# Enter-tainer/oavif

Hardware: AMD Instinct MI355X
Metric: ssimulacra2_megapixels_per_sec (higher is better)
Workload: dtype f32; 1 GPU; ssimulacra2 score of one 3840x2160 RGB8 (ref, dist) pair per step per GPU (BASELINE configs[1]); steps rotate over 16 distinct pairs per GPU = 796 MB of frames resident in HBM (> the 256 MiB Infinity Cache); width=3840, height=2160, distinct_pairs_per_gpu=16, parallelism=single gpu, streams_per_gpu=2

## Files before the change

### include/ssimu2_hip_internal.h

```cpp
#ifndef SSIMU2_HIP_INTERNAL_H_
#define SSIMU2_HIP_INTERNAL_H_

#include "ssimu2_hip.h"

#ifdef __cplusplus
extern "C" {
#endif
#if defined(__GNUC__)
#pragma GCC visibility push(default)
#endif

enum { SSIMU2_DEBUG_LIN_REF = 0, SSIMU2_DEBUG_LIN_DIST = 1, SSIMU2_DEBUG_XYB_REF = 2, SSIMU2_DEBUG_REF_BLUR = 3,
       SSIMU2_DEBUG_RG_H = 4, SSIMU2_DEBUG_RG_V = 5 };
int ssimu2_debug_download(ssimu2_ctx* ctx, int what, int scale, uint32_t w, uint32_t h, float* out,
                          uint32_t* out_w, uint32_t* out_h);

int ssimu2_time_device(ssimu2_ctx* ctx, const void* d_ref, const void* d_dist, uint32_t w,
                       uint32_t h, int iters, float* out_ms_total, double* out_score);

enum { SSIMU2_STAGE_PYRAMID = 0, SSIMU2_STAGE_MARCH = 1, SSIMU2_STAGE_FINALIZE = 2 };
int ssimu2_time_stage(ssimu2_ctx* ctx, const void* d_ref, const void* d_dist, uint32_t w, uint32_t h,
                      int stage, int iters, float* out_ms_avg);

int ssimu2_time_march_rotating(ssimu2_ctx* ctx, const void* const* d_refs, const void* const* d_dists,
                               int npairs, uint32_t w, uint32_t h, int iters, float* out_ms_avg);

int ssimu2_measure_read_stream(ssimu2_ctx* ctx, size_t bytes, int iters, double* out_gbps);

int ssimu2_instr_set_segment_rows(ssimu2_ctx* ctx, int rows_scale0, int rows_other_scales);
int ssimu2_instr_cache_reference_blur(ssimu2_ctx* ctx, int enabled);
enum {
    SSIMU2_MARCH_NONE = 0,
    SSIMU2_MARCH_PAIR_U8 = 1,
    SSIMU2_MARCH_REFBLUR_U8 = 2,
    SSIMU2_MARCH_PAIR_LIN = 3,
    SSIMU2_MARCH_REFBLUR_LIN = 4,
    SSIMU2_MARCH_PAIR_BATCH = 5,
    SSIMU2_MARCH_REFBLUR_BATCH = 6
};
int ssimu2_instr_last_march(ssimu2_ctx* ctx, int* out_kind);
int ssimu2_instr_set_batch_segment_rows(ssimu2_ctx* ctx, int rows_scale0);
int ssimu2_instr_batch_segment_rows(ssimu2_ctx* ctx, uint32_t w, uint32_t h, int scale, int* out_rows);
int ssimu2_time_blur_stage_rotating(ssimu2_ctx* ctx, const void* const* d_frames, int nframes, uint32_t w,
                                    uint32_t h, int iters, float* out_ms_avg, double* out_bytes_per_launch);
int ssimu2_time_kernels(ssimu2_ctx* ctx, const void* d_ref, const void* const* d_refs, const void* const* d_dists, int n,
                        uint32_t w, uint32_t h, int iters, float* out_ms_avg, int* out_launches, float* out_ms_wall_timed,
                        float* out_ms_wall_plain);
int ssimu2_instr_placed_streams(ssimu2_ctx* ctx, int* out_n);
int ssimu2_instr_rg_stop_after_scale(ssimu2_ctx* ctx, int scale);

#if defined(__GNUC__)
#pragma GCC visibility pop
#endif
#ifdef __cplusplus
}
#endif
#endif
```

### oavif_amd/csrc/ssimu2_instrument.hip

```cpp
#define SSIMU2_INSTRUMENTED_BUILD 1
#include "ssimu2_hip.hip"

#include <vector>

#include "../../include/ssimu2_hip_internal.h"

namespace ssimu2 {

__global__ __launch_bounds__(256) void k_read_stream(const uint4* __restrict__ src, size_t n16,
                                                     uint32_t* __restrict__ sink) {
    const size_t chunk = (n16 + gridDim.x - 1) / gridDim.x;
    const size_t lo = (size_t)blockIdx.x * chunk;
    const size_t hi = lo + chunk < n16 ? lo + chunk : n16;
    size_t i = lo + threadIdx.x;
    uint4 acc = make_uint4(0, 0, 0, 0);
    for (; i + 768 < hi; i += 1024) {
        const uint4 a = src[i], b = src[i + 256], c = src[i + 512], d = src[i + 768];
        acc.x ^= a.x ^ b.x ^ c.x ^ d.x;
        acc.y ^= a.y ^ b.y ^ c.y ^ d.y;
        acc.z ^= a.z ^ b.z ^ c.z ^ d.z;
        acc.w ^= a.w ^ b.w ^ c.w ^ d.w;
    }
    for (; i < hi; i += 256) {
        const uint4 a = src[i];
        acc.x ^= a.x; acc.y ^= a.y; acc.z ^= a.z; acc.w ^= a.w;
    }
    const uint32_t v = acc.x ^ acc.y ^ acc.z ^ acc.w;
    if (v == 0x9E3779B9u) *sink = v;
}

}

extern "C" {

int ssimu2_instr_set_segment_rows(ssimu2_ctx* c, int rows_scale0, int rows_other_scales) {
    REMOTE_REFUSE(c, "ssimu2_instr_set_segment_rows");
    if (!c) return SSIMU2_ERR_INVALID_ARG;
    if ((rows_scale0 != 0 && (rows_scale0 < 8 || rows_scale0 > 160)) ||
        (rows_other_scales != 0 && (rows_other_scales < 8 || rows_other_scales > 160)))
        return c->fail(SSIMU2_ERR_INVALID_ARG, "segment rows must be 0 (default rule) or 8..160");
    HIP_TRY(c, hipSetDevice(c->device));
    HIP_TRY(c, hipStreamSynchronize(c->stream));
    c->seg_rows_override = rows_scale0;
    c->seg_rows_tail_override = rows_other_scales;
    release_frame_groups(c);
    return SSIMU2_OK;
}

int ssimu2_instr_set_batch_segment_rows(ssimu2_ctx* c, int rows_scale0) {
    REMOTE_REFUSE(c, "ssimu2_instr_set_batch_segment_rows");
    if (!c) return SSIMU2_ERR_INVALID_ARG;
    if (rows_scale0 != 0 && rows_scale0 != -1 && (rows_scale0 < 8 || rows_scale0 > 160))
        return c->fail(SSIMU2_ERR_INVALID_ARG, "batch segment rows must be 0 (the rule), -1 (the single-score rule) or 8..160");
    HIP_TRY(c, hipSetDevice(c->device));
    HIP_TRY(c, hipStreamSynchronize(c->stream));
    c->batch_seg_override = rows_scale0;
    return SSIMU2_OK;
}

int ssimu2_instr_batch_segment_rows(ssimu2_ctx* c, uint32_t w, uint32_t h, int scale, int* out_rows) {
    REMOTE_REFUSE(c, "ssimu2_instr_batch_segment_rows");
    if (!c || !out_rows || scale < 0 || scale >= kNumScales || w == 0 || h == 0) return SSIMU2_ERR_INVALID_ARG;
    *out_rows = batch_seg_rows(c, make_pyramid(w, h), scale);
    return SSIMU2_OK;
}

int ssimu2_instr_placed_streams(ssimu2_ctx* c, int* out_n) {
    REMOTE_REFUSE(c, "ssimu2_instr_placed_streams");
    if (!c || !out_n) return SSIMU2_ERR_INVALID_ARG;
    *out_n = pool_size(c->device);
    return SSIMU2_OK;
}

int ssimu2_instr_rg_stop_after_scale(ssimu2_ctx* c, int scale) {
    REMOTE_REFUSE(c, "ssimu2_instr_rg_stop_after_scale");
    if (!c) return SSIMU2_ERR_INVALID_ARG;
    c->rg_dbg_scale = scale < 0 || scale >= kNumScales ? -1 : scale;
    return SSIMU2_OK;
}

int ssimu2_instr_cache_reference_blur(ssimu2_ctx* c, int enabled) {
    REMOTE_REFUSE(c, "ssimu2_instr_cache_reference_blur");
    if (!c) return SSIMU2_ERR_INVALID_ARG;
    c->cache_ref_blur = enabled != 0;
    c->ref.drop();
    return SSIMU2_OK;
}

int ssimu2_instr_last_march(ssimu2_ctx* c, int* out_kind) {
    REMOTE_REFUSE(c, "ssimu2_instr_last_march");
    if (!c || !out_kind) return SSIMU2_ERR_INVALID_ARG;
    *out_kind = c->last_march;
    return SSIMU2_OK;
}

int ssimu2_debug_download(ssimu2_ctx* c, int what, int scale, uint32_t w, uint32_t h, float* out,
                          uint32_t* out_w, uint32_t* out_h) {
    REMOTE_REFUSE(c, "ssimu2_debug_download");
    if (!c || !out) return SSIMU2_ERR_INVALID_ARG;
    if (w == 0 || h == 0) return c->fail(SSIMU2_ERR_INVALID_ARG, "zero image dimension");
    const Pyramid p = make_pyramid(w, h);
    const float* src = nullptr;
    if ((what == SSIMU2_DEBUG_LIN_REF || what == SSIMU2_DEBUG_LIN_DIST) && scale == 0) {
        const bool r = what == SSIMU2_DEBUG_LIN_REF;
        const void* planes = r ? c->hbd.lin0_ref.p : c->hbd.lin0_dist.p;
        if (!planes || p.nscales < 1 || (r ? c->lin0_ref_w : c->lin0_dist_w) != w ||
            (r ? c->lin0_ref_h : c->lin0_dist_h) != h)
            return c->fail(SSIMU2_ERR_INVALID_ARG, "no 16-bit scale-0 planes of that frame from the last score");
        src = (const float*)planes;
    } else if (what == SSIMU2_DEBUG_LIN_REF || what == SSIMU2_DEBUG_LIN_DIST) {
        if (scale < 1 || scale >= p.nscales || !c->frame.lin_ref.p) return c->fail(SSIMU2_ERR_INVALID_ARG, "no such level");
        src = (what == SSIMU2_DEBUG_LIN_REF ? c->frame.lin_ref : c->frame.lin_dist).as<float>() + p.lin_off[scale];
    } else if (what == SSIMU2_DEBUG_XYB_REF) {
        if (scale < 0 || scale >= p.nscales || !c->cache.xyb.p || !c->ref.have || c->ref.w != w || c->ref.h != h)
            return c->fail(SSIMU2_ERR_INVALID_ARG, "no cached reference XYB for that level");
        src = c->cache.xyb.as<float>() + xyb_off(p, scale);
    } else if (what == SSIMU2_DEBUG_RG_H || what == SSIMU2_DEBUG_RG_V) {
        if (scale < 0 || scale >= p.nscales || scale != c->rg_dbg_scale || !c->rg.dbg.p || !c->rg.planes.p)
            return c->fail(SSIMU2_ERR_INVALID_ARG, "no recursive-blur planes kept for that scale");
        const size_t pitch = (size_t)rg_pitch(p.w[scale]), wd = (size_t)p.w[scale], ht = (size_t)p.h[scale];
        const size_t nd = pitch * ht, n1 = wd * ht;
        if (24 * nd * sizeof(float) > c->rg.dbg.cap) return c->fail(SSIMU2_ERR_INVALID_ARG, "recursive-blur planes are of another frame size");
        HIP_TRY(c, hipSetDevice(c->device));
        HIP_TRY(c, hipStreamSynchronize(c->stream));
        auto plane = [&](float* dst, const float* src) {
            return hipMemcpy2D(dst, wd * sizeof(float), src, pitch * sizeof(float), wd * sizeof(float), ht, hipMemcpyDeviceToHost);
        };
        if (what == SSIMU2_DEBUG_RG_H) {
            for (int k = 0; k < 15; ++k) HIP_TRY(c, plane(out + (size_t)k * n1, c->rg.dbg.as<float>() + (size_t)k * nd));
        } else {
            const float* cache = c->rg.planes.as<float>() + 6 * rg_plane_off(p, p.nscales) + 6 * rg_plane_off(p, scale);
            const float* pass = c->rg.dbg.as<float>() + 15 * nd;
            for (int ch = 0; ch < 3; ++ch) {
                for (int k = 0; k < 2; ++k)
                    HIP_TRY(c, plane(out + (size_t)rg_plane15(true, ch, k) * n1, cache + (size_t)(ch * 2 + k) * nd));
                for (int k = 0; k < 3; ++k)
                    HIP_TRY(c, plane(out + (size_t)rg_plane15(false, ch, k) * n1, pass + (size_t)(ch * 3 + k) * nd));
            }
        }
        if (out_w) *out_w = (uint32_t)p.w[scale];
        if (out_h) *out_h = (uint32_t)p.h[scale];
        return SSIMU2_OK;
    } else if (what == SSIMU2_DEBUG_REF_BLUR) {
        if (scale < 0 || scale >= p.nscales || !c->cache.blur.p || !c->ref.have || c->ref.w != w || c->ref.h != h)
            return c->fail(SSIMU2_ERR_INVALID_ARG, "no cached reference blur for that level");
        src = c->cache.blur.as<float>() + xyb_off(p, scale);
    } else {
        return c->fail(SSIMU2_ERR_INVALID_ARG, "bad `what`");
    }
    HIP_TRY(c, hipSetDevice(c->device));
    HIP_TRY(c, hipStreamSynchronize(c->stream));
    const size_t n = (size_t)3 * p.w[scale] * p.h[scale];
    HIP_TRY(c, hipMemcpy(out, src, n * sizeof(float), hipMemcpyDeviceToHost));
    if (out_w) *out_w = (uint32_t)p.w[scale];
    if (out_h) *out_h = (uint32_t)p.h[scale];
    return SSIMU2_OK;
}

int ssimu2_time_device(ssimu2_ctx* c, const void* d_ref, const void* d_dist, uint32_t w,
                       uint32_t h, int iters, float* out_ms_total, double* out_score) {
    REMOTE_REFUSE(c, "ssimu2_time_device");
    int rc = check_args(c, d_ref, d_dist, w, h);
    if (rc) return rc;
    if (iters <= 0 || !out_ms_total) return c->fail(SSIMU2_ERR_INVALID_ARG, "bad iters/out");
    HIP_TRY(c, hipSetDevice(c->device));
    if ((rc = ensure_capacity(c, w, h))) return rc;
    c->ref.drop();
    HIP_TRY(c, hipEventRecord(c->ev0, c->stream));
    for (int i = 0; i < iters; ++i)
        if ((rc = enqueue_score(c, (const uint8_t*)d_ref, (const uint8_t*)d_dist, w, h, false)))
            return rc;
    HIP_TRY(c, hipEventRecord(c->ev1, c->stream));
    double score = 0.0;
    if ((rc = ssimu2_wait(c, &score))) return rc;
    HIP_TRY(c, hipEventSynchronize(c->ev1));
    HIP_TRY(c, hipEventElapsedTime(out_ms_total, c->ev0, c->ev1));
    if (out_score) *out_score = score;
    return SSIMU2_OK;
}

}

namespace {

template <class F>
struct AtExit {
    F f;
    ~AtExit() { f(); }
};
template <class F>
AtExit(F) -> AtExit<F>;
auto scratch_guard(ssimu2_ctx* c, DevBuf& b) {
    return AtExit{[c, &b] { (void)hipStreamSynchronize(c->stream), b.release(); }};
}

template <class T>
std::vector<T> host_array(int n) {
    try {
        return std::vector<T>((size_t)n);
    } catch (const std::bad_alloc&) {
        return {};
    }
}

template <class F>
hipError_t timed_loop(ssimu2_ctx* c, int warm, int iters, float* ms, F&& fn) {
    for (int j = 0; j < warm; ++j) fn(j);
    hipError_t e = hipEventRecord(c->ev0, c->stream);
    for (int j = 0; j < iters && e == hipSuccess; ++j) fn(j);
    if (e == hipSuccess) e = hipEventRecord(c->ev1, c->stream);
    if (e == hipSuccess) e = hipGetLastError();
    if (e == hipSuccess) e = hipEventSynchronize(c->ev1);
    if (e == hipSuccess) e = hipEventElapsedTime(ms, c->ev0, c->ev1);
    return e;
}

}

extern "C" {

int ssimu2_time_stage(ssimu2_ctx* c, const void* d_ref, const void* d_dist, uint32_t w, uint32_t h,
                      int stage, int iters, float* out_ms_avg) {
    REMOTE_REFUSE(c, "ssimu2_time_stage");
    int rc = check_args(c, d_ref, d_dist, w, h);
    if (rc) return rc;
    if (iters <= 0 || !out_ms_avg) return c->fail(SSIMU2_ERR_INVALID_ARG, "bad iters/out");
    double score;
    if ((rc = ssimu2_score_rgb8_device(c, d_ref, d_dist, w, h, &score))) return rc;
    const Pyramid p = make_pyramid(w, h);
    MarchPlan mp;
    FinalizeArgs fa;
    const int blocks = build_plans(c, p, march_seg_rows, score_sources(c, d_ref, d_dist, false), &mp, &fa);
    if (stage < 0 || stage > 2) return c->fail(SSIMU2_ERR_INVALID_ARG, "bad stage");
    const uint8_t* frames[2] = {(const uint8_t*)d_ref, (const uint8_t*)d_dist};
    float* lin[2] = {c->frame.lin_ref.as<float>(), c->frame.lin_dist.as<float>()};
    float ms = 0.f;
    const hipError_t e = timed_loop(c, 0, iters, &ms, [&](int) {
        if (stage == SSIMU2_STAGE_PYRAMID) launch_pyramid(c, p, 2, frames, lin);
        else if (stage == SSIMU2_STAGE_FINALIZE) launch(k_finalize, dim3(1), dim3(1024), 0, c->stream, fa, c->d_result);
        else if (blocks > 0) launch(k_march, dim3(blocks), dim3(MARCH_THREADS), 0, c->stream, mp);
    });
    if (e != hipSuccess) return c->fail(SSIMU2_ERR_HIP, "stage timing", e);
    *out_ms_avg = ms / (float)iters;
    return SSIMU2_OK;
}

int ssimu2_time_march_rotating(ssimu2_ctx* c, const void* const* d_refs, const void* const* d_dists,
                               int npairs, uint32_t w, uint32_t h, int iters, float* out_ms_avg) {
    REMOTE_REFUSE(c, "ssimu2_time_march_rotating");
    if (!c) return SSIMU2_ERR_INVALID_ARG;
    if (!d_refs || !d_dists || npairs <= 0 || npairs > 64 || iters <= 0 || !out_ms_avg)
        return c->fail(SSIMU2_ERR_INVALID_ARG, "bad pairs/iters/out");
    int rc = check_args(c, d_refs[0], d_dists[0], w, h);
    if (rc) return rc;
    HIP_TRY(c, hipSetDevice(c->device));
    if ((rc = ensure_capacity(c, w, h))) return rc;
    c->ref.drop();
    const Pyramid p = make_pyramid(w, h);
    const size_t lin_floats = p.lin_total + 4;
    DevBuf lin;
    const auto free_lin = scratch_guard(c, lin);
    rc = grow(c, lin, (size_t)npairs * 2 * lin_floats * sizeof(float), "hipMalloc(rotating pyramids)");
    if (rc) return rc;
    std::vector<MarchPlan> plans = host_array<MarchPlan>(npairs);
    if (plans.empty()) return c->fail(SSIMU2_ERR_OOM, "plans");
// ... 164 lines not shown
```

### oavif_amd/csrc/ssimu2_kernels.h

```cpp
#pragma once

#include <hip/hip_runtime.h>
#include <stdint.h>

#include "../../include/ssimu2_hip.h"
#include "ssimu2_div_rn.h"

namespace ssimu2 {

constexpr int kNumScales = SSIMU2_NUM_SCALES;
constexpr int kStats = SSIMU2_STATS_PER_SCALE;

constexpr float kC2 = 0.0009f;
constexpr float kM00 = 0.30f, kM01 = 0.622f, kM02 = 0.078f;
constexpr float kM10 = 0.23f, kM11 = 0.692f, kM12 = 0.078f;
constexpr float kM20 = 0.24342268924547819f, kM21 = 0.20476744424496821f,
                kM22 = 0.55180986650955360f;
constexpr float kOpsinBias = 0.0037930732552754493f;

struct DevConst {
    float lut[256];
    float taps[5];
    float cbrt_bias;
    float rg_n2[3];
    float rg_d1[3];
    double weights[108];
};
__constant__ DevConst c_k;


template <bool GUARD>
__host__ __device__ __forceinline__ float cbrt_repro(float x) {
    uint32_t i = __builtin_bit_cast(uint32_t, x);
#ifdef __HIP_DEVICE_COMPILE__
    i = __umulhi(i, 0x55555556u);
#else
    i = i / 3u;
#endif
    i = 0x54A21D2Au - i;
    float y = __builtin_bit_cast(float, i);
    float t = x * y;
    t = t * y;
    t = t * y;
    const float e = 1.0f - t;
    float p = fmaf(e, 14.0f / 81.0f, 2.0f / 9.0f);
    p = fmaf(p, e, 1.0f / 3.0f);
    p = p * e;
    y = fmaf(y, p, y);
    const float y2 = y * y;
    float c = x * y2;
    const float r = fmaf(c * c, c, -x);
    c = fmaf(r, y2 * (-1.0f / 3.0f), c);
    return GUARD ? (x > 0.0f ? c : 0.0f) : c;
}

__device__ __forceinline__ void opsin_mix(float r, float g, float b, float (&lms)[3]) {
    lms[0] = fmaf(kM00, r, fmaf(kM01, g, fmaf(kM02, b, kOpsinBias)));
    lms[1] = fmaf(kM10, r, fmaf(kM11, g, fmaf(kM12, b, kOpsinBias)));
    lms[2] = fmaf(kM20, r, fmaf(kM21, g, fmaf(kM22, b, kOpsinBias)));
}
template <bool CLAMP>
__device__ __forceinline__ void mixed_to_xyb(const float (&lms)[3], float (&v)[3]) {
    float l = lms[0], m = lms[1], s = lms[2];
    if (CLAMP) {
        l = fmaxf(l, 0.0f);
        m = fmaxf(m, 0.0f);
        s = fmaxf(s, 0.0f);
    }
    const float cb = c_k.cbrt_bias;
    l = cbrt_repro<CLAMP>(l) - cb;
    m = cbrt_repro<CLAMP>(m) - cb;
    s = cbrt_repro<CLAMP>(s) - cb;
    const float x = 0.5f * (l - m), y = 0.5f * (l + m);
    v[2] = (s - y) + 0.55f;
    v[0] = fmaf(x, 14.0f, 0.42f);
    v[1] = y + 0.01f;
}
__device__ __forceinline__ void linear_to_xyb(float r, float g, float b, float& X, float& Y, float& B) {
    float lms[3], v[3];
    opsin_mix(r, g, b, lms);
    mixed_to_xyb<true>(lms, v);
    B = v[2];
    X = v[0];
    Y = v[1];
}

__device__ __forceinline__ float fir9(float c, float s1, float s2, float s3, float s4, float w0,
                                      float w1, float w2, float w3, float w4) {
    float acc = w0 * c;
    acc = fmaf(w1, s1, acc);
    acc = fmaf(w2, s2, acc);
    acc = fmaf(w3, s3, acc);
    acc = fmaf(w4, s4, acc);
    return acc;
}

__device__ __forceinline__ float ssim_term(float mu1, float mu2, float s11, float s22, float s12) {
    const float mu11 = mu1 * mu1, mu22 = mu2 * mu2, mu12 = mu1 * mu2;
    const float dm = mu1 - mu2;
    const float num_m = fmaf(-dm, dm, 1.0f);
    const float num_s = fmaf(2.0f, s12 - mu12, kC2);
    const float denom_s = ((s11 - mu11) + (s22 - mu22)) + kC2;
    const float d = 1.0f - div_rn(num_m * num_s, denom_s);
    return fmaxf(d, 0.0f);
}
template <bool RN>
__device__ __forceinline__ float edge_quotient(float mu1, float mu2, float r1, float r2) {
    const float ea = fabsf(r2 - mu2), eb = fabsf(r1 - mu1);
    return RN ? div_rn(ea - eb, 1.0f + eb) : (ea - eb) * __builtin_amdgcn_rcpf(1.0f + eb);
}
template <typename Put>
__device__ __forceinline__ void six_terms(float d, float e, Put put) {
    const float art = fmaxf(e, 0.0f), det = fmaxf(-e, 0.0f);
    const float d2 = d * d, a2 = art * art, t2 = det * det;
    put(0, d);
    put(1, d2 * d2);
    put(2, art);
    put(3, a2 * a2);
    put(4, det);
    put(5, t2 * t2);
}

__device__ __forceinline__ double wave_sum(double v) {
#pragma unroll
    for (int off = 32; off > 0; off >>= 1) v += __shfl_down(v, off, 64);
    return v;
}

struct PyrBandArgs {
    const uint8_t* in[2];
    float* out[2][5];
    float* xyb0[2];
    int w[6], h[6];
    int opitch[6];
    int nlevels;
    int bands_x, bands_y, nframes;
    unsigned* zero4;
};

struct PyrHbdArgs {
    const uint8_t* in[2];
    uint32_t pitch[2];
    const float* tab[2];
    uint32_t maxv[2];
    float* lin0[2];
};

constexpr int PYR_THREADS = 512;
constexpr int PYR_TX = PYR_THREADS / 8;
constexpr int PYR_BAND_W = 4 * PYR_TX, PYR_BAND_H = 32;
constexpr int PYR_BAND_LDS_FLOATS = 3 * 8 * PYR_TX + 3 * 4 * (PYR_TX / 2) + 3 * 2 * (PYR_TX / 4);

__device__ __forceinline__ float box4(float p00, float p01, float p10, float p11) {
    float sum = p00;
    sum += p01;
    sum += p10;
    sum += p11;
    return sum * 0.25f;
}

__device__ __forceinline__ void pyr_store_xyb(float* out, size_t n, size_t at, const float (&lin)[3]) {
    float X, Y, B;
    linear_to_xyb(lin[0], lin[1], lin[2], X, Y, B);
    out[at] = X;
    out[n + at] = Y;
    out[2 * n + at] = B;
}

template <bool XYB>
__device__ __forceinline__ void pyr_lds_level(const float* src, int sw, int sh, int wa, int ha, float* dst_tile,
                                              int dw_tile, int dh_tile, float* out, int wo, int ho, int po, int ox0,
                                              int oy0, int lx, int ly) {
    const int ox = ox0 + lx, oy = oy0 + ly;
    float v[3] = {0.f, 0.f, 0.f};
    if (ox < wo && oy < ho) {
        const int xa = 2 * lx, xb = min(2 * ox + 1, wa - 1) - 2 * ox0;
        const int ya = 2 * ly, yb = min(2 * oy + 1, ha - 1) - 2 * oy0;
        const size_t n = (size_t)po * ho;
#pragma unroll
        for (int c = 0; c < 3; ++c) {
            const float* p = src + c * sw * sh;
            v[c] = box4(p[ya * sw + xa], p[ya * sw + xb], p[yb * sw + xa], p[yb * sw + xb]);
            if (!XYB) out[c * n + (size_t)oy * po + ox] = v[c];
        }
        if (XYB) pyr_store_xyb(out, n, (size_t)oy * po + ox, v);
    }
    if (dst_tile) {
#pragma unroll
        for (int c = 0; c < 3; ++c) dst_tile[(c * dh_tile + ly) * dw_tile + lx] = v[c];
    }
}

template <int CH>
__device__ __forceinline__ void pyr_load16(const PyrHbdArgs& hb, int f, int w0, int h0, int X0, int Y0, bool inside,
                                           float (&lin)[4][4][3]) {
    const uint8_t* base = hb.in[f];
    const uint32_t pitch = hb.pitch[f], maxv = hb.maxv[f];
    const float* tab = hb.tab[f];
    uint32_t s[4][4][3];
    if (inside) {
        uint32_t raw[4][2 * CH];
#pragma unroll
        for (int j = 0; j < 4; ++j) {
            const uint8_t* p = base + (size_t)(Y0 + j) * pitch + (size_t)X0 * (2 * CH);
#pragma unroll
            for (int k = 0; k < 2 * CH; ++k) __builtin_memcpy(&raw[j][k], p + 4 * k, 4);
        }
#pragma unroll
        for (int j = 0; j < 4; ++j)
#pragma unroll
            for (int i = 0; i < 4; ++i)
#pragma unroll
                for (int c = 0; c < 3; ++c) {
                    const int e = CH * i + c;
                    s[j][i][c] = (raw[j][e >> 1] >> (16 * (e & 1))) & 0xFFFFu;
                }
    } else {
#pragma unroll
        for (int j = 0; j < 4; ++j) {
            const uint8_t* row = base + (size_t)min(Y0 + j, h0 - 1) * pitch;
#pragma unroll
            for (int i = 0; i < 4; ++i) {
                const uint16_t* p = (const uint16_t*)(row + (size_t)min(X0 + i, w0 - 1) * (2 * CH));
#pragma unroll
                for (int c = 0; c < 3; ++c) s[j][i][c] = p[c];
            }
        }
    }
#pragma unroll
    for (int j = 0; j < 4; ++j)
#pragma unroll
        for (int i = 0; i < 4; ++i)
#pragma unroll
            for (int c = 0; c < 3; ++c) lin[j][i][c] = tab[min(s[j][i][c], maxv)];
}

template <bool XYB, int CH16 = 0, bool BATCH = false>
__device__ __forceinline__ void pyramid_band(const PyrBandArgs& a, int band, const float* lut, float* lds,
                                             const PyrHbdArgs* hb = nullptr, size_t in_off = 0, size_t out_off = 0) {
    const int t = threadIdx.x;
    const int per_frame = a.bands_x * a.bands_y;
    const int f = band / per_frame;
    const int r = band - f * per_frame;
    const int by = r / a.bands_x, bx = r - by * a.bands_x;
    const int w0 = a.w[0], h0 = a.h[0], w1 = a.w[1], h1 = a.h[1];
    constexpr int TX = PYR_TX;
    float* s2 = lds;
    float* s3 = s2 + 3 * 8 * TX;
    float* s4 = s3 + 3 * 4 * (TX / 2);
    const int tx = t % TX, ty = t / TX;
    const int X0 = bx * PYR_BAND_W + 4 * tx, Y0 = by * PYR_BAND_H + 4 * ty;
    float l1[2][2][3];
#pragma unroll
    for (int j = 0; j < 2; ++j)
#pragma unroll
        for (int i = 0; i < 2; ++i)
#pragma unroll
            for (int c = 0; c < 3; ++c) l1[j][i][c] = 0.f;
    if (X0 < w0 && Y0 < h0) {
        const uint8_t* base = a.in[f];
        if constexpr (BATCH) base += in_off;
        uint32_t raw[4][3];
        float lin16[4][4][3];
        const bool inside = X0 + 3 < w0 && Y0 + 3 < h0;
        if constexpr (CH16 != 0) {
            pyr_load16<CH16>(*hb, f, w0, h0, X0, Y0, inside, lin16);
        } else if (inside) {
#pragma unroll
            for (int j = 0; j < 4; ++j) {
                const uint8_t* p = base + ((size_t)(Y0 + j) * w0 + X0) * 3;
#pragma unroll
                for (int k = 0; k < 3; ++k) __builtin_memcpy(&raw[j][k], p + 4 * k, 4);
            }
        } else {
#pragma unroll
            for (int j = 0; j < 4; ++j) {
                const int y = min(Y0 + j, h0 - 1);
                uint8_t b[12];
#pragma unroll
                for (int i = 0; i < 4; ++i) {
                    const uint8_t* p = base + ((size_t)y * w0 + min(X0 + i, w0 - 1)) * 3;
                    b[3 * i] = p[0];
                    b[3 * i + 1] = p[1];
                    b[3 * i + 2] = p[2];
                }
#pragma unroll
                for (int k = 0; k < 3; ++k)
                    raw[j][k] = (uint32_t)b[4 * k] | ((uint32_t)b[4 * k + 1] << 8) | ((uint32_t)b[4 * k + 2] << 16) |
                                ((uint32_t)b[4 * k + 3] << 24);
            }
        }
#define PYR_LIN(j, i, c) \
    (CH16 ? lin16[j][i][c] : lut[(raw[j][(3 * (i) + (c)) >> 2] >> (8 * ((3 * (i) + (c)) & 3))) & 255u])
        const int p1 = a.opitch[1];
        const size_t n1 = (size_t)p1 * h1;
#pragma unroll
        for (int j = 0; j < 2; ++j) {
#pragma unroll
            for (int i = 0; i < 2; ++i) {
                const int ox = (X0 >> 1) + i, oy = (Y0 >> 1) + j;
#pragma unroll
                for (int c = 0; c < 3; ++c)
                    l1[j][i][c] = box4(PYR_LIN(2 * j, 2 * i, c), PYR_LIN(2 * j, 2 * i + 1, c),
                                       PYR_LIN(2 * j + 1, 2 * i, c), PYR_LIN(2 * j + 1, 2 * i + 1, c));
                if (ox < w1 && oy < h1 && (!XYB || a.nlevels >= 1)) {
                    float* o = a.out[f][0];
                    if constexpr (BATCH) o += out_off;
                    if (XYB) {
                        pyr_store_xyb(o, n1, (size_t)oy * p1 + ox, l1[j][i]);
                    } else {
#pragma unroll
                        for (int c = 0; c < 3; ++c) o[c * n1 + (size_t)oy * p1 + ox] = l1[j][i][c];
                    }
                }
            }
        }
        if constexpr (CH16 != 0 && !XYB) {
            const size_t n0 = (size_t)w0 * h0;
            float* o = hb->lin0[f];
#pragma unroll
            for (int j = 0; j < 4; ++j) {
                if (inside) {
                    const size_t at = (size_t)(Y0 + j) * w0 + X0;
#pragma unroll
                    for (int c = 0; c < 3; ++c) {
                        const float px[4] = {lin16[j][0][c], lin16[j][1][c], lin16[j][2][c], lin16[j][3][c]};
                        __builtin_memcpy(o + c * n0 + at, px, 16);
                    }
                } else if (Y0 + j < h0) {
#pragma unroll
                    for (int i = 0; i < 4; ++i)
                        if (X0 + i < w0) {
#pragma unroll
                            for (int c = 0; c < 3; ++c) o[c * n0 + (size_t)(Y0 + j) * w0 + X0 + i] = lin16[j][i][c];
                        }
                }
            }
        }
        if (XYB) {
            const int p0 = a.opitch[0];
            const size_t n0 = (size_t)p0 * h0;
            float* o = a.xyb0[f];
#pragma unroll
            for (int j = 0; j < 4; ++j) {
                float px[3][4];
#pragma unroll
                for (int i = 0; i < 4; ++i) {
                    linear_to_xyb(PYR_LIN(j, i, 0), PYR_LIN(j, i, 1), PYR_LIN(j, i, 2), px[0][i], px[1][i], px[2][i]);
                }
                if (inside) {
                    const size_t at = (size_t)(Y0 + j) * p0 + X0;
#pragma unroll
                    for (int c = 0; c < 3; ++c) __builtin_memcpy(o + c * n0 + at, px[c], 16);
                } else if (Y0 + j < h0) {
#pragma unroll
                    for (int i = 0; i < 4; ++i)
                        if (X0 + i < w0) {
#pragma unroll
                            for (int c = 0; c < 3; ++c) o[c * n0 + (size_t)(Y0 + j) * p0 + X0 + i] = px[c][i];
                        }
                }
            }
        }
#undef PYR_LIN
    }
    if (a.nlevels < 2) return;
    {
        const int w2 = a.w[2], h2 = a.h[2];
        const int ox = X0 >> 2, oy = Y0 >> 2;
        float v[3] = {0.f, 0.f, 0.f};
        if (ox < w2 && oy < h2) {
            const int ib = min(2 * ox + 1, w1 - 1) - 2 * ox, jb = min(2 * oy + 1, h1 - 1) - 2 * oy;
            const int p2 = a.opitch[2];
            const size_t n2 = (size_t)p2 * h2;
            float* o = a.out[f][1];
            if constexpr (BATCH) o += out_off;
#pragma unroll
            for (int c = 0; c < 3; ++c) {
                const float p01 = ib ? l1[0][1][c] : l1[0][0][c];
                const float p10 = jb ? l1[1][0][c] : l1[0][0][c];
                const float p11 = jb ? (ib ? l1[1][1][c] : l1[1][0][c]) : (ib ? l1[0][1][c] : l1[0][0][c]);
                v[c] = box4(l1[0][0][c], p01, p10, p11);
                if (!XYB) o[c * n2 + (size_t)oy * p2 + ox] = v[c];
            }
            if (XYB) pyr_store_xyb(o, n2, (size_t)oy * p2 + ox, v);
        }
#pragma unroll
        for (int c = 0; c < 3; ++c) s2[(c * 8 + ty) * TX + tx] = v[c];
    }
    if (a.nlevels < 3) return;
    __syncthreads();
    if (t < 4 * (TX / 2))
        pyr_lds_level<XYB>(s2, TX, 8, a.w[2], a.h[2], s3, TX / 2, 4, BATCH ? a.out[f][2] + out_off : a.out[f][2], a.w[3], a.h[3], a.opitch[3], bx * (TX / 2), by * 4,
                      t % (TX / 2), t / (TX / 2));
    if (a.nlevels < 4) return;
    __syncthreads();
    if (t < 2 * (TX / 4))
        pyr_lds_level<XYB>(s3, TX / 2, 4, a.w[3], a.h[3], s4, TX / 4, 2, BATCH ? a.out[f][3] + out_off : a.out[f][3], a.w[4], a.h[4], a.opitch[4], bx * (TX / 4), by * 2,
                      t % (TX / 4), t / (TX / 4));
    if (a.nlevels < 5) return;
    __syncthreads();
    if (t < TX / 8)
        pyr_lds_level<XYB>(s4, TX / 4, 2, a.w[4], a.h[4], nullptr, 0, 0, BATCH ? a.out[f][4] + out_off : a.out[f][4], a.w[5], a.h[5], a.opitch[5], bx * (TX / 8), by, t, 0);
}

__global__ __launch_bounds__(PYR_THREADS) void k_pyramid_bands(PyrBandArgs a) {
    __shared__ float s_lut[256];
    __shared__ float s_tiles[PYR_BAND_LDS_FLOATS];
    if (threadIdx.x < 256) s_lut[threadIdx.x] = c_k.lut[threadIdx.x];
    __syncthreads();
    pyramid_band<false>(a, (int)blockIdx.x, s_lut, s_tiles);
}

struct PyrBatchArgs {
    PyrBandArgs a;
    size_t in_stride;
    size_t out_stride;
};
__global__ __launch_bounds__(PYR_THREADS) void k_pyramid_bands_batch(PyrBatchArgs b) {
    __shared__ float s_lut[256];
    __shared__ float s_tiles[PYR_BAND_LDS_FLOATS];
    if (threadIdx.x < 256) s_lut[threadIdx.x] = c_k.lut[threadIdx.x];
    __syncthreads();
    const int per_item = b.a.bands_x * b.a.bands_y * b.a.nframes;
    const int item = (int)blockIdx.x / per_item;
    pyramid_band<false, 0, true>(b.a, (int)blockIdx.x - item * per_item, s_lut, s_tiles, nullptr, (size_t)item * b.in_stride,
                        (size_t)item * b.out_stride);
}

__global__ __launch_bounds__(PYR_THREADS) void k_pyramid_bands_xyb(PyrBandArgs a) {
    __shared__ float s_lut[256];
    __shared__ float s_tiles[PYR_BAND_LDS_FLOATS];
    if (threadIdx.x < 256) s_lut[threadIdx.x] = c_k.lut[threadIdx.x];
    if (blockIdx.x == 0 && threadIdx.x < 4 && a.zero4) a.zero4[threadIdx.x] = 0u;
    __syncthreads();
    pyramid_band<true>(a, (int)blockIdx.x, s_lut, s_tiles);
}

template <int CH>
__global__ __launch_bounds__(PYR_THREADS) void k_pyramid_bands16(PyrBandArgs a, PyrHbdArgs hb) {
    __shared__ float s_tiles[PYR_BAND_LDS_FLOATS];
    pyramid_band<false, CH>(a, (int)blockIdx.x, nullptr, s_tiles, &hb);
}

template <int CH>
__global__ __launch_bounds__(PYR_THREADS) void k_pyramid_bands_xyb16(PyrBandArgs a, PyrHbdArgs hb) {
    __shared__ float s_tiles[PYR_BAND_LDS_FLOATS];
    if (blockIdx.x == 0 && threadIdx.x < 4 && a.zero4) a.zero4[threadIdx.x] = 0u;
    __syncthreads();
    pyramid_band<true, CH>(a, (int)blockIdx.x, nullptr, s_tiles, &hb);
}

constexpr int RAD = 4;
constexpr int MW = 120;
constexpr int MRW = MW + 8;
constexpr int MHALF = MW / 2;
constexpr int RING = 16;
constexpr int AHEAD = 3;
constexpr int GROUP = 3;
constexpr int MARCH_THREADS = 512;
constexpr int CONV_WAVES = 2;

typedef float f2 __attribute__((ext_vector_type(2)));
constexpr int RING_ROW = 3 * MRW;

struct MarchPlan {
    int nscales;
    int blk_end[kNumScales];
    int w[kNumScales], h[kNumScales], seg[kNumScales], nstrips[kNumScales], nblocks[kNumScales];
    const void* ref[kNumScales];
    const void* dist[kNumScales];
    const float* ref_xyb[kNumScales];
    float* ref_s11[kNumScales];
    double* part[kNumScales];
};

enum { MARCH_PAIR = 0, MARCH_REFBLUR = 1, MARCH_EMIT = 2, MARCH_MAP = 3 };

constexpr int RB_AHEAD = 6;
struct MarchRefBlur {
    float* s11;
    int pitch;
    int rows_left;
    bool active;
    float ps11[9];
};

struct MapCoef {
    float c[kNumScales][kStats];
};

__device__ __forceinline__ float map_density(const float (&t)[6], const float (&mc)[6]) {
    float v = mc[0] * t[0];
#pragma unroll
    for (int k = 1; k < 6; ++k) v = fmaf(mc[k], t[k], v);
    return v;
}
__device__ __forceinline__ int term_stat(int c, int k) { return k < 2 ? c * 2 + k : 6 + c * 4 + (k - 2); }

struct MarchCursor {
    const uint8_t* base;
    uint32_t off;
    size_t plane;
    int pitch;
    uint32_t shift;
};

template <bool U8>
__device__ __forceinline__ MarchCursor march_cursor(const void* base, int w, int h, int gxc) {
    MarchCursor c;
    c.plane = (size_t)w * h * 4;
    c.pitch = U8 ? w * 3 : w * 4;
    const bool last_col = U8 && gxc == w - 1;
    c.shift = last_col ? 8u : 0u;
    c.base = (const uint8_t*)base;
    c.off = (uint32_t)gxc * (U8 ? 3u : 4u) - (last_col ? 1u : 0u);
    return c;
}

template <bool U8>
__device__ __forceinline__ void march_load(uint32_t (&raw)[3], MarchCursor& c, int row) {
    const uint8_t* p = c.base + (size_t)(uint32_t)row * (uint32_t)c.pitch;
    asm volatile("" : "+v"(c.off));
    const uint32_t off = c.off;
    if (U8) {
        uint32_t d;
        __builtin_memcpy(&d, p + off, 4);
        raw[0] = d;
    } else {
        raw[0] = *(const uint32_t*)(p + off);
        raw[1] = *(const uint32_t*)((p + c.plane) + off);
        raw[2] = *(const uint32_t*)((p + 2 * c.plane) + off);
    }
}

__device__ __forceinline__ void march_lut(const float* lut, uint32_t d, uint32_t shift, float (&lin)[3]) {
    d >>= shift;
    lin[0] = lut[d & 255u];
    lin[1] = lut[(d >> 8) & 255u];
    lin[2] = lut[(d >> 16) & 255u];
}

template <bool U8, int MODE, bool LIN0 = false, bool BATCH = false>
__device__ __forceinline__ void march_convert_rows(f2 (*ring)[3][MRW], const float* lut,
                                                   const MarchPlan& plan, int sc, int w, int h, int x0,
                                                   int y0, int steps, int ngroups, int col, size_t off0 = 0,
                                                   size_t off1 = 0) {
    constexpr bool CACHED = MODE == MARCH_REFBLUR || MODE == MARCH_EMIT;
    constexpr bool TWO = MODE != MARCH_EMIT;
    constexpr bool LUT0 = U8 && !CACHED;
    const int gx = x0 - RAD + col;
    const bool col_ok = gx >= 0 && gx < w;
    const bool all_cols = x0 - RAD >= 0 && x0 - RAD + MRW <= w;
    const int gxc = min(max(gx, 0), w - 1);
    MarchCursor c0 = CACHED ? march_cursor<false>(plan.ref_xyb[sc], w, h, gxc)
                            : march_cursor<U8>(plan.ref[sc], w, h, gxc);
    MarchCursor c1 = march_cursor<U8>(plan.dist[sc], w, h, gxc);
    if constexpr (BATCH) {
        if (!CACHED) c0.base += off0;
        c1.base += off1;
    }
    int load_row = y0 - RAD;
    constexpr int NG = 2;
    constexpr int QD = NG * GROUP;
    uint32_t raw0[QD][3], raw1[QD][3];
    float lin0[3] = {0.f, 0.f, 0.f}, lin1[3] = {0.f, 0.f, 0.f};
#define MARCH_LOAD(J)                                                      \
    {                                                                      \
        const int lrow_ = min(max(load_row, 0), h - 1);       \
        if (CACHED) march_load<false>(raw0[J], c0, lrow_);                 \
        else march_load<U8>(raw0[J], c0, lrow_);                           \
        if (TWO) march_load<U8>(raw1[J], c1, lrow_);                       \
        ++load_row;                                                        \
    }
#define MARCH_LUT(J)                                                             \
    if (U8) {                                                                    \
        if (LUT0) march_lut(lut, raw0[J][0], c0.shift, lin0);                    \
        if (TWO) march_lut(lut, raw1[J][0], c1.shift, lin1);                     \
    }
#define MARCH_PUT(J, R)                                                                        \
    {                                                                                          \
           \
                              \
        const bool rok_ = (unsigned)(y0 - RAD + (R)) < (unsigned)h;                            \
        float a_[3] = {0.f, 0.f, 0.f}, b_[3] = {0.f, 0.f, 0.f};                                \
        float m0_[3], m1_[3];                                                                  \
        if (!CACHED) {                                                                         \
            if (U8) opsin_mix(lin0[0], lin0[1], lin0[2], m0_);                                 \
// ... 493 lines not shown
```

Baseline: 54620 MP/s.

## Issue pyramid band loads before LUT staging and use 32-bit offset addressing

Restructures the pyramid band kernel so each thread's global pixel loads are issued before the LUT is copied into LDS and before the barrier, letting the load latency overlap the LUT fill. Store and load addresses are rebuilt as a row base plus a 32-bit lane offset, hidden from the optimizer with an asm barrier, to cut 64-bit address arithmetic. When aligned, level-1 stores are paired into float2, and the pyramid kernels raise wave priority with s_setprio. The batch debug download path gains new enum values for inspecting batched linear planes. The risks are extra register pressure from holding raw loads across the barrier, and an empty-asm offset trick that only holds while offsets fit in 32 bits.

```diff
diff --git a/include/ssimu2_hip_internal.h b/include/ssimu2_hip_internal.h
--- a/include/ssimu2_hip_internal.h
+++ b/include/ssimu2_hip_internal.h
@@ -11,7 +11,8 @@
 #endif
 
 enum { SSIMU2_DEBUG_LIN_REF = 0, SSIMU2_DEBUG_LIN_DIST = 1, SSIMU2_DEBUG_XYB_REF = 2, SSIMU2_DEBUG_REF_BLUR = 3,
-       SSIMU2_DEBUG_RG_H = 4, SSIMU2_DEBUG_RG_V = 5 };
+       SSIMU2_DEBUG_RG_H = 4, SSIMU2_DEBUG_RG_V = 5,
+       SSIMU2_DEBUG_BATCH_LIN_REF = 6, SSIMU2_DEBUG_BATCH_LIN_DIST = 7, SSIMU2_DEBUG_BATCH_ITEM = 8 };
 int ssimu2_debug_download(ssimu2_ctx* ctx, int what, int scale, uint32_t w, uint32_t h, float* out,
                           uint32_t* out_w, uint32_t* out_h);
 
diff --git a/oavif_amd/csrc/ssimu2_instrument.hip b/oavif_amd/csrc/ssimu2_instrument.hip
--- a/oavif_amd/csrc/ssimu2_instrument.hip
+++ b/oavif_amd/csrc/ssimu2_instrument.hip
@@ -111,6 +111,15 @@
     } else if (what == SSIMU2_DEBUG_LIN_REF || what == SSIMU2_DEBUG_LIN_DIST) {
         if (scale < 1 || scale >= p.nscales || !c->frame.lin_ref.p) return c->fail(SSIMU2_ERR_INVALID_ARG, "no such level");
         src = (what == SSIMU2_DEBUG_LIN_REF ? c->frame.lin_ref : c->frame.lin_dist).as<float>() + p.lin_off[scale];
+    } else if (what >= SSIMU2_DEBUG_BATCH_LIN_REF) {
+        const int kind = SSIMU2_DEBUG_BATCH_LIN_REF + (what - SSIMU2_DEBUG_BATCH_LIN_REF) % SSIMU2_DEBUG_BATCH_ITEM;
+        const size_t item = (size_t)(what - SSIMU2_DEBUG_BATCH_LIN_REF) / SSIMU2_DEBUG_BATCH_ITEM;
+        const DevBuf& buf = kind == SSIMU2_DEBUG_BATCH_LIN_REF ? c->batch.lin_ref : c->batch.lin_dist;
+        const size_t lin_stride = (p.lin_total + 3) & ~(size_t)3;
+        if (kind > SSIMU2_DEBUG_BATCH_LIN_DIST || scale < 1 || scale >= p.nscales || item >= c->batch_n || !buf.p ||
+            (size_t)c->batch_n * lin_stride * sizeof(float) > buf.cap)
+            return c->fail(SSIMU2_ERR_INVALID_ARG, "no such level of such an item of the last batch");
+        src = buf.as<float>() + item * lin_stride + p.lin_off[scale];
     } else if (what == SSIMU2_DEBUG_XYB_REF) {
         if (scale < 0 || scale >= p.nscales || !c->cache.xyb.p || !c->ref.have || c->ref.w != w || c->ref.h != h)
             return c->fail(SSIMU2_ERR_INVALID_ARG, "no cached reference XYB for that level");
diff --git a/oavif_amd/csrc/ssimu2_kernels.h b/oavif_amd/csrc/ssimu2_kernels.h
--- a/oavif_amd/csrc/ssimu2_kernels.h
+++ b/oavif_amd/csrc/ssimu2_kernels.h
@@ -159,12 +159,18 @@
     return sum * 0.25f;
 }
 
-__device__ __forceinline__ void pyr_store_xyb(float* out, size_t n, size_t at, const float (&lin)[3]) {
+template <typename T>
+__device__ __forceinline__ T* pyr_at(T* row, uint32_t at) {
+    asm volatile("" : "+v"(at));
+    return (T*)((const char*)row + at);
+}
+
+__device__ __forceinline__ void pyr_store_xyb(float* row, size_t n, uint32_t at, const float (&lin)[3]) {
     float X, Y, B;
     linear_to_xyb(lin[0], lin[1], lin[2], X, Y, B);
-    out[at] = X;
-    out[n + at] = Y;
-    out[2 * n + at] = B;
+    *pyr_at(row, at) = X;
+    *pyr_at(row + n, at) = Y;
+    *pyr_at(row + 2 * n, at) = B;
 }
 
 template <bool XYB>
@@ -177,13 +183,15 @@
         const int xa = 2 * lx, xb = min(2 * ox + 1, wa - 1) - 2 * ox0;
         const int ya = 2 * ly, yb = min(2 * oy + 1, ha - 1) - 2 * oy0;
         const size_t n = (size_t)po * ho;
+        float* origin = out + (size_t)oy0 * po + ox0;
+        const uint32_t at = 4u * (uint32_t)(ly * po + lx);
 #pragma unroll
         for (int c = 0; c < 3; ++c) {
             const float* p = src + c * sw * sh;
             v[c] = box4(p[ya * sw + xa], p[ya * sw + xb], p[yb * sw + xa], p[yb * sw + xb]);
-            if (!XYB) out[c * n + (size_t)oy * po + ox] = v[c];
-        }
-        if (XYB) pyr_store_xyb(out, n, (size_t)oy * po + ox, v);
+            if (!XYB) *pyr_at(origin + c * n, at) = v[c];
+        }
+        if (XYB) pyr_store_xyb(origin, n, at, v);
     }
     if (dst_tile) {
 #pragma unroll
@@ -236,7 +244,7 @@
 }
 
 template <bool XYB, int CH16 = 0, bool BATCH = false>
-__device__ __forceinline__ void pyramid_band(const PyrBandArgs& a, int band, const float* lut, float* lds,
+__device__ __forceinline__ void pyramid_band(const PyrBandArgs& a, int band, float* lut, float* lds,
                                              const PyrHbdArgs* hb = nullptr, size_t in_off = 0, size_t out_off = 0) {
     const int t = threadIdx.x;
     const int per_frame = a.bands_x * a.bands_y;
@@ -245,102 +253,118 @@
     const int by = r / a.bands_x, bx = r - by * a.bands_x;
     const int w0 = a.w[0], h0 = a.h[0], w1 = a.w[1], h1 = a.h[1];
     constexpr int TX = PYR_TX;
+    static_assert(TX == 64, "one thread row per wave: ty below is read from lane 0");
     float* s2 = lds;
     float* s3 = s2 + 3 * 8 * TX;
     float* s4 = s3 + 3 * 4 * (TX / 2);
-    const int tx = t % TX, ty = t / TX;
-    const int X0 = bx * PYR_BAND_W + 4 * tx, Y0 = by * PYR_BAND_H + 4 * ty;
-    float l1[2][2][3];
-#pragma unroll
-    for (int j = 0; j < 2; ++j)
-#pragma unroll
-        for (int i = 0; i < 2; ++i)
-#pragma unroll
-            for (int c = 0; c < 3; ++c) l1[j][i][c] = 0.f;
-    if (X0 < w0 && Y0 < h0) {
-        const uint8_t* base = a.in[f];
-        if constexpr (BATCH) base += in_off;
-        uint32_t raw[4][3];
+    const int tx = t % TX, ty = __builtin_amdgcn_readfirstlane(t / TX);
+    const int XB = bx * PYR_BAND_W;
+    const int X0 = XB + 4 * tx, Y0 = by * PYR_BAND_H + 4 * ty;
+    const bool work = X0 < w0 && Y0 < h0;
+    const bool inside = X0 + 3 < w0 && Y0 + 3 < h0;
+    uint32_t raw[4][3];
+    if constexpr (CH16 == 0) {
+        const float entry = c_k.lut[t & 255];
+        if (work) {
+            const uint8_t* base = a.in[f];
+            if constexpr (BATCH) base += in_off;
+            if (inside) {
+                const uint8_t* row0 = base + ((size_t)Y0 * w0 + XB) * 3;
+                const uint32_t at = 12u * tx;
+#pragma unroll
+                for (int j = 0; j < 4; ++j) {
+                    const uint8_t* p = pyr_at(row0 + (size_t)j * w0 * 3, at);
+#pragma unroll
+                    for (int k = 0; k < 3; ++k) __builtin_memcpy(&raw[j][k], p + 4 * k, 4);
+                }
+            } else {
+#pragma unroll
+                for (int j = 0; j < 4; ++j) {
+                    const uint8_t* row = base + ((size_t)min(Y0 + j, h0 - 1) * w0 + XB) * 3;
+                    uint8_t b[12];
+#pragma unroll
+                    for (int i = 0; i < 4; ++i) {
+                        const uint8_t* p = pyr_at(row, 3u * (uint32_t)(min(X0 + i, w0 - 1) - XB));
+                        b[3 * i] = p[0];
+                        b[3 * i + 1] = p[1];
+                        b[3 * i + 2] = p[2];
+                    }
+#pragma unroll
+                    for (int k = 0; k < 3; ++k)
+                        raw[j][k] = (uint32_t)b[4 * k] | ((uint32_t)b[4 * k + 1] << 8) | ((uint32_t)b[4 * k + 2] << 16) |
+                                    ((uint32_t)b[4 * k + 3] << 24);
+                }
+            }
+        }
+        if (t < 256) lut[t] = entry;
+        __syncthreads();
+    }
+    float v2[3] = {0.f, 0.f, 0.f};
+    if (work) {
         float lin16[4][4][3];
-        const bool inside = X0 + 3 < w0 && Y0 + 3 < h0;
-        if constexpr (CH16 != 0) {
-            pyr_load16<CH16>(*hb, f, w0, h0, X0, Y0, inside, lin16);
-        } else if (inside) {
-#pragma unroll
-            for (int j = 0; j < 4; ++j) {
-                const uint8_t* p = base + ((size_t)(Y0 + j) * w0 + X0) * 3;
-#pragma unroll
-                for (int k = 0; k < 3; ++k) __builtin_memcpy(&raw[j][k], p + 4 * k, 4);
-            }
-        } else {
-#pragma unroll
-            for (int j = 0; j < 4; ++j) {
-                const int y = min(Y0 + j, h0 - 1);
-                uint8_t b[12];
-#pragma unroll
-                for (int i = 0; i < 4; ++i) {
-                    const uint8_t* p = base + ((size_t)y * w0 + min(X0 + i, w0 - 1)) * 3;
-                    b[3 * i] = p[0];
-                    b[3 * i + 1] = p[1];
-                    b[3 * i + 2] = p[2];
-                }
-#pragma unroll
-                for (int k = 0; k < 3; ++k)
-                    raw[j][k] = (uint32_t)b[4 * k] | ((uint32_t)b[4 * k + 1] << 8) | ((uint32_t)b[4 * k + 2] << 16) |
-                                ((uint32_t)b[4 * k + 3] << 24);
-            }
-        }
+        if constexpr (CH16 != 0) pyr_load16<CH16>(*hb, f, w0, h0, X0, Y0, inside, lin16);
 #define PYR_LIN(j, i, c) \
     (CH16 ? lin16[j][i][c] : lut[(raw[j][(3 * (i) + (c)) >> 2] >> (8 * ((3 * (i) + (c)) & 3))) & 255u])
+        float l1[2][2][3];
         const int p1 = a.opitch[1];
         const size_t n1 = (size_t)p1 * h1;
+        float* o1 = a.out[f][0];
+        if constexpr (BATCH) o1 += out_off;
+        const int ox1 = X0 >> 1, oy1 = Y0 >> 1;
+        const bool pairs = !XYB && (p1 & 1) == 0 && ((uintptr_t)o1 & 7) == 0;
 #pragma unroll
         for (int j = 0; j < 2; ++j) {
 #pragma unroll
-            for (int i = 0; i < 2; ++i) {
-                const int ox = (X0 >> 1) + i, oy = (Y0 >> 1) + j;
+            for (int i = 0; i < 2; ++i)
 #pragma unroll
                 for (int c = 0; c < 3; ++c)
                     l1[j][i][c] = box4(PYR_LIN(2 * j, 2 * i, c), PYR_LIN(2 * j, 2 * i + 1, c),
                                        PYR_LIN(2 * j + 1, 2 * i, c), PYR_LIN(2 * j + 1, 2 * i + 1, c));
-                if (ox < w1 && oy < h1 && (!XYB || a.nlevels >= 1)) {
-                    float* o = a.out[f][0];
-                    if constexpr (BATCH) o += out_off;
-                    if (XYB) {
-                        pyr_store_xyb(o, n1, (size_t)oy * p1 + ox, l1[j][i]);
-                    } else {
-#pragma unroll
-                        for (int c = 0; c < 3; ++c) o[c * n1 + (size_t)oy * p1 + ox] = l1[j][i][c];
-                    }
-                }
-            }
-        }
-        if constexpr (CH16 != 0 && !XYB) {
-            const size_t n0 = (size_t)w0 * h0;
-            float* o = hb->lin0[f];
-#pragma unroll
-            for (int j = 0; j < 4; ++j) {
-                if (inside) {
-                    const size_t at = (size_t)(Y0 + j) * w0 + X0;
-#pragma unroll
-                    for (int c = 0; c < 3; ++c) {
-                        const float px[4] = {lin16[j][0][c], lin16[j][1][c], lin16[j][2][c], lin16[j][3][c]};
-                        __builtin_memcpy(o + c * n0 + at, px, 16);
-                    }
-                } else if (Y0 + j < h0) {
-#pragma unroll
-                    for (int i = 0; i < 4; ++i)
-                        if (X0 + i < w0) {
-#pragma unroll
-                            for (int c = 0; c < 3; ++c) o[c * n0 + (size_t)(Y0 + j) * w0 + X0 + i] = lin16[j][i][c];
+            if (oy1 + j < h1 && (!XYB || a.nlevels >= 1)) {
+                float* row = o1 + (size_t)(oy1 + j) * p1 + (XB >> 1);
+                const uint32_t at = 8u * tx;
+                if (XYB) {
+#pragma unroll
+                    for (int i = 0; i < 2; ++i)
+                        if (ox1 + i < w1) pyr_store_xyb(row, n1, at + 4 * i, l1[j][i]);
+                } else if (pairs && ox1 + 1 < w1) {
+#pragma unroll
+                    for (int c = 0; c < 3; ++c) *(float2*)pyr_at(row + c * n1, at) = make_float2(l1[j][0][c], l1[j][1][c]);
+                } else {
+#pragma unroll
+                    for (int i = 0; i < 2; ++i)
+                        if (ox1 + i < w1) {
+#pragma unroll
+                            for (int c = 0; c < 3; ++c) *pyr_at(row + c * n1, at + 4 * i) = l1[j][i][c];
                         }
                 }
             }
         }
+        if constexpr (CH16 != 0 && !XYB) {
+            const size_t n0 = (size_t)w0 * h0;
+#pragma unroll
+            for (int j = 0; j < 4; ++j) {
+                float* row = hb->lin0[f] + (size_t)(Y0 + j) * w0 + XB;
+                const uint32_t at = 16u * tx;
+                if (inside) {
+#pragma unroll
+                    for (int c = 0; c < 3; ++c) {
+                        const float px[4] = {lin16[j][0][c], lin16[j][1][c], lin16[j][2][c], lin16[j][3][c]};
+                        __builtin_memcpy(pyr_at(row + c * n0, at), px, 16);
+                    }
+                } else if (Y0 + j < h0) {
+#pragma unroll
+                    for (int i = 0; i < 4; ++i)
+                        if (X0 + i < w0) {
+#pragma unroll
+                            for (int c = 0; c < 3; ++c) *pyr_at(row + c * n0, at + 4 * i) = lin16[j][i][c];
+                        }
+                }
+            }
+        }
         if (XYB) {
             const int p0 = a.opitch[0];
             const size_t n0 = (size_t)p0 * h0;
-            float* o = a.xyb0[f];
 #pragma unroll
             for (int j = 0; j < 4; ++j) {
                 float px[3][4];
@@ -348,46 +372,45 @@
                 for (int i = 0; i < 4; ++i) {
                     linear_to_xyb(PYR_LIN(j, i, 0), PYR_LIN(j, i, 1), PYR_LIN(j, i, 2), px[0][i], px[1][i], px[2][i]);
                 }
+                float* row = a.xyb0[f] + (size_t)(Y0 + j) * p0 + XB;
+                const uint32_t at = 16u * tx;
                 if (inside) {
-                    const size_t at = (size_t)(Y0 + j) * p0 + X0;
-#pragma unroll
-                    for (int c = 0; c < 3; ++c) __builtin_memcpy(o + c * n0 + at, px[c], 16);
+#pragma unroll
+                    for (int c = 0; c < 3; ++c) __builtin_memcpy(pyr_at(row + c * n0, at), px[c], 16);
                 } else if (Y0 + j < h0) {
 #pragma unroll
                     for (int i = 0; i < 4; ++i)
                         if (X0 + i < w0) {
 #pragma unroll
-                            for (int c = 0; c < 3; ++c) o[c * n0 + (size_t)(Y0 + j) * p0 + X0 + i] = px[c][i];
+                            for (int c = 0; c < 3; ++c) *pyr_at(row + c * n0, at + 4 * i) = px[c][i];
                         }
                 }
             }
         }
 #undef PYR_LIN
-    }
-    if (a.nlevels < 2) return;
-    {
         const int w2 = a.w[2], h2 = a.h[2];
         const int ox = X0 >> 2, oy = Y0 >> 2;
-        float v[3] = {0.f, 0.f, 0.f};
-        if (ox < w2 && oy < h2) {
+        if (a.nlevels >= 2 && ox < w2 && oy < h2) {
             const int ib = min(2 * ox + 1, w1 - 1) - 2 * ox, jb = min(2 * oy + 1, h1 - 1) - 2 * oy;
             const int p2 = a.opitch[2];
             const size_t n2 = (size_t)p2 * h2;
-            float* o = a.out[f][1];
-            if constexpr (BATCH) o += out_off;
+            float* row = a.out[f][1] + (size_t)oy * p2 + (XB >> 2);
+            if constexpr (BATCH) row += out_off;
+            const uint32_t at = 4u * tx;
 #pragma unroll
             for (int c = 0; c < 3; ++c) {
                 const float p01 = ib ? l1[0][1][c] : l1[0][0][c];
                 const float p10 = jb ? l1[1][0][c] : l1[0][0][c];
                 const float p11 = jb ? (ib ? l1[1][1][c] : l1[1][0][c]) : (ib ? l1[0][1][c] : l1[0][0][c]);
-                v[c] = box4(l1[0][0][c], p01, p10, p11);
-                if (!XYB) o[c * n2 + (size_t)oy * p2 + ox] = v[c];
+                v2[c] = box4(l1[0][0][c], p01, p10, p11);
+                if (!XYB) *pyr_at(row + c * n2, at) = v2[c];
             }
-            if (XYB) pyr_store_xyb(o, n2, (size_t)oy * p2 + ox, v);
-        }
-#pragma unroll
-        for (int c = 0; c < 3; ++c) s2[(c * 8 + ty) * TX + tx] = v[c];
-    }
+            if (XYB) pyr_store_xyb(row, n2, at, v2);
+        }
+    }
+    if (a.nlevels < 2) return;
+#pragma unroll
+    for (int c = 0; c < 3; ++c) s2[(c * 8 + ty) * TX + tx] = v2[c];
     if (a.nlevels < 3) return;
     __syncthreads();
     if (t < 4 * (TX / 2))
@@ -404,11 +427,12 @@
         pyr_lds_level<XYB>(s4, TX / 4, 2, a.w[4], a.h[4], nullptr, 0, 0, BATCH ? a.out[f][4] + out_off : a.out[f][4], a.w[5], a.h[5], a.opitch[5], bx * (TX / 8), by, t, 0);
 }
 
+__device__ __forceinline__ void pyr_issue_first() { __builtin_amdgcn_s_setprio(3); }
+
 __global__ __launch_bounds__(PYR_THREADS) void k_pyramid_bands(PyrBandArgs a) {
     __shared__ float s_lut[256];
     __shared__ float s_tiles[PYR_BAND_LDS_FLOATS];
-    if (threadIdx.x < 256) s_lut[threadIdx.x] = c_k.lut[threadIdx.x];
-    __syncthreads();
+    pyr_issue_first();
     pyramid_band<false>(a, (int)blockIdx.x, s_lut, s_tiles);
 }
 
@@ -420,8 +444,7 @@
 __global__ __launch_bounds__(PYR_THREADS) void k_pyramid_bands_batch(PyrBatchArgs b) {
     __shared__ float s_lut[256];
     __shared__ float s_tiles[PYR_BAND_LDS_FLOATS];
-    if (threadIdx.x < 256) s_lut[threadIdx.x] = c_k.lut[threadIdx.x];
-    __syncthreads();
+    pyr_issue_first();
     const int per_item = b.a.bands_x * b.a.bands_y * b.a.nframes;
     const int item = (int)blockIdx.x / per_item;
     pyramid_band<false, 0, true>(b.a, (int)blockIdx.x - item * per_item, s_lut, s_tiles, nullptr, (size_t)item * b.in_stride,
@@ -431,9 +454,7 @@
 __global__ __launch_bounds__(PYR_THREADS) void k_pyramid_bands_xyb(PyrBandArgs a) {
     __shared__ float s_lut[256];
     __shared__ float s_tiles[PYR_BAND_LDS_FLOATS];
-    if (threadIdx.x < 256) s_lut[threadIdx.x] = c_k.lut[threadIdx.x];
     if (blockIdx.x == 0 && threadIdx.x < 4 && a.zero4) a.zero4[threadIdx.x] = 0u;
-    __syncthreads();
     pyramid_band<true>(a, (int)blockIdx.x, s_lut, s_tiles);
 }
 
```

Result: faster. 56200 MP/s (median of 6 runs) (+2.9%).
